# EternalEvan/InstaRevive

Measured on AMD Instinct MI355X. Metric: 512->2048 one-step SR images/sec, higher is better.
Workload: dtype bf16

## Files before the change

### instarevive_amd/csrc/conv_s1.hip

```cpp
#include <stdlib.h>
#include <type_traits>
#include <utility>
#include "agpr256.h"
#include "common.h"
#include "kernels.h"
#include "conv_s1_epi.h"

namespace cs1 {
constexpr int TH = 16, TW = 32, HWD = TW + 2, HP = (TH + 2) * HWD;
constexpr int BK = 32, ROWB = 64;
constexpr int H_Q = (HP + 15) / 16;
constexpr int HALO_BYTES = H_Q * 1024;
constexpr int H_I = 10;
constexpr int BN = 128, WT_BYTES = BN * ROWB;
constexpr int NSB = 4;
constexpr int NHB = 3;
constexpr int W_OFF = NHB * HALO_BYTES;
constexpr int LDS_MAIN = W_OFF + NSB * WT_BYTES;
static_assert(cs1e::BYTES <= HALO_BYTES, "epilogue slabs + reduction area must fit one halo buffer");
constexpr int LDS_BYTES = LDS_MAIN;
template <int NTAP>
struct Geo {
    static constexpr int K = NTAP == 9 ? 3 : 2, HWD = TW + K - 1, HP = (TH + K - 1) * HWD, H_Q = (HP + 15) / 16, H_I = (H_Q + 3) / 4;
};
static_assert(Geo<9>::H_Q == H_Q && Geo<9>::H_I == H_I && Geo<4>::H_Q == 36 && Geo<4>::H_I == 9, "halo piece counts");
constexpr int nh(int ntap, int t) { return ntap == 9 ? (t < 4 ? 2 : (t < 6 ? 1 : 0)) : (t == 0 ? 3 : 2); }
constexpr int nh_first(int ntap, int t) { return ntap == 9 ? (t < 4 ? 2 * t : (t < 6 ? 4 + t : 0)) : (t == 0 ? 0 : 1 + 2 * t); }
constexpr int hkey(int hx) { return ((hx >> 2) & 1) << 1; }
}

#ifdef IR_S1_STAMPS
__device__ unsigned long long g_s1_stamps[1024 * 8];
#define IR_S1_T(v) const unsigned long long v = __builtin_amdgcn_s_memrealtime()
#define IR_S1_ACC(k, a, b) do { if (tid == 0) g_s1_stamps[blockIdx.x * 8 + (k)] += (b) - (a); } while (0)
#else
#define IR_S1_T(v) do { } while (0)
#define IR_S1_ACC(k, a, b) do { } while (0)
#endif

typedef __attribute__((address_space(3))) void* cs1_lds_t;
template <int LO>
IR_DEVINL void cs1_mfma(bf16x8 w, bf16x8 px) {
    asm volatile("v_mfma_f32_16x16x32_bf16 a[%c2:%c3], %0, %1, a[%c2:%c3]" ::"v"(w), "v"(px), "n"(LO), "n"(LO + 3));
}

template <int UP, int NTAP, bool NORM = false, int EFULL = 0>
__global__ __launch_bounds__(256, 1) void conv_halo_s1_kernel(IGemmParams p, int tiles_y, int tiles_x, int total_vb) {
    static_assert(!NORM || (UP == 0 && NTAP == 9), "the in-kernel GroupNorm form exists for the plain 9-tap conv");
#if defined(__HIP_DEVICE_COMPILE__)
    using namespace cs1;
    using G = Geo<NTAP>;
    constexpr int K = G::K, HWD = G::HWD, HP = G::HP, H_Q = G::H_Q, H_I = G::H_I;
    constexpr bool PH = NTAP == 4;
    constexpr int NP_OFF = LDS_MAIN, NP_SLOT = 2 * 512 * 4;
    __shared__ __attribute__((aligned(1024))) unsigned char smem[NORM ? LDS_MAIN + 2 * NP_SLOT : LDS_BYTES];
    const int tid = threadIdx.x, lane = tid & 63, wid = tid >> 6;
    const int wu = __builtin_amdgcn_readfirstlane(wid);
    const int c16 = lane & 15, kq = lane >> 4;
    const int NT = p.Cout_pad / BN;
    const int MT = p.NB * tiles_y * tiles_x * (PH ? 4 : 1);
    const int Hc = UP ? 2 * p.H : p.H, Wc = UP ? 2 * p.W : p.W;
    const int chunks = p.Cin / BK;

    struct Tile { int img, trem, oy0, ox0, n0, dy, dx; };
    auto decode = [&](int bid, Tile& t) -> bool {
        const int xcd = bid & 7, jb = bid >> 3;
        const int mt = (jb / NT) * 8 + xcd, nt = jb % NT;
        if (bid >= total_vb || mt >= MT) return false;
        t.n0 = nt * BN;
        const int per_img = tiles_y * tiles_x * (PH ? 4 : 1);
        t.img = mt / per_img;
        t.trem = mt - t.img * per_img;
        const int ph = PH ? (t.trem & 3) : 0, tile = PH ? (t.trem >> 2) : t.trem;
        t.dy = ph >> 1; t.dx = ph & 1;
        const int ty = tile / tiles_x, tx = tile - ty * tiles_x;
        t.oy0 = ty * TH; t.ox0 = tx * TW;
        return true;
    };
    constexpr uint32_t OOB = 0xfffffff0u;
    auto tile_base = [&](const Tile& t) -> const bf16_t* {
        const int by = max(t.oy0 - 1 + t.dy, 0) >> UP;
        return p.in + ((long)t.img * p.H + by) * p.W * p.in_cs;
    };
    auto describe = [&](const Tile& t, uint32_t (&hp)[H_I], uint32_t (&wp)[2]) {
        const int by = max(t.oy0 - 1 + t.dy, 0) >> UP;
#pragma unroll
        for (int i = 0; i < H_I; ++i) {
            const int q = min(wu + 4 * i, H_Q - 1);
            const int hpix = q * 16 + (lane >> 2);
            const int hy = hpix / HWD, hx = hpix - hy * HWD;
            const int cy = t.oy0 + hy - 1 + t.dy, cx = t.ox0 + hx - 1 + t.dx;
            const bool ok = hpix < HP && cy >= 0 && cy < Hc && cx >= 0 && cx < Wc;
            const int iy = min(max(cy, 0), Hc - 1) >> UP, ix = min(max(cx, 0), Wc - 1) >> UP;
            const uint32_t sw = (uint32_t)((lane & 3) ^ hkey(hx));
            hp[i] = ok ? (uint32_t)(((iy - by) * p.W + ix) * p.in_cs) * 2u + sw * 16u : OOB;
        }
#pragma unroll
        for (int i = 0; i < 2; ++i) {
            const int row = (wu + 4 * i) * 16 + (lane >> 2);
            wp[i] = (uint32_t)(((PH ? (2 * t.dy + t.dx) * p.Cout_pad : 0) + t.n0 + row) * (int)p.wgt_rs) * 2u + (uint32_t)((lane & 3) ^ hkey(row)) * 16u;
        }
    };
    auto rsrc_of = [&](const void* base) { return __builtin_amdgcn_make_buffer_rsrc(const_cast<void*>(base), 0, 0x7fffffff, 0x00020000); };
    const __amdgpu_buffer_rsrc_t w_rsrc = rsrc_of(p.wgt);
    const uint32_t lds0 = lds_addr(smem);
    uint32_t hrd[K];
#pragma unroll
    for (int kx = 0; kx < K; ++kx) {
        const int hx = kx + c16;
        hrd[kx] = lds0 + ((4 * wid) * HWD + hx) * ROWB + ((kq ^ hkey(hx)) << 4);
    }
    const uint32_t wrd = lds0 + W_OFF + c16 * ROWB + ((kq ^ hkey(c16)) << 4);
    bf16x8 fw[2][8], fp[NORM ? 1 : 2][NORM ? 1 : 8];
    bf16x8 fq[3];

    Tile cur, nxt;
    int bid = blockIdx.x;
    while (bid < total_vb && !decode(bid, cur)) bid += gridDim.x;
    if (bid >= total_vb) return;
    uint32_t h_ptr[H_I], h_nxt[H_I], w_ptr[2], w_nxt[2];
    describe(cur, h_ptr, w_ptr);
    const bf16_t* base_cur = tile_base(cur);
    const bf16_t* base_nxt = base_cur;

    auto halo_issue = [&](auto ic, int ci, int buf) {
        constexpr int i = decltype(ic)::value;
        const int q = min(wu + 4 * i, H_Q - 1);
        const bool mine = ci < chunks;
        __builtin_amdgcn_raw_ptr_buffer_load_lds(rsrc_of(mine ? base_cur : base_nxt), (cs1_lds_t)(smem + buf * HALO_BYTES + q * 1024), 16,
                                                 (int)(mine ? h_ptr[i] : h_nxt[i]), (mine ? ci : ci - chunks) * (BK * 2), 0, 0);
    };
    auto w_issue = [&](int chunk, int tap, bool mine, int slot) {
        const int koff = tap * p.Cin + chunk * BK;
#pragma unroll
        for (int i = 0; i < 2; ++i)
            __builtin_amdgcn_raw_ptr_buffer_load_lds(w_rsrc, (cs1_lds_t)(smem + W_OFF + slot * WT_BYTES + (wu + 4 * i) * 1024), 16,
                                                     (int)(mine ? w_ptr[i] : w_nxt[i]), koff * 2, 0, 0);
    };

    int hb3 = 0;
    [&]<int... I>(std::integer_sequence<int, I...>) { (halo_issue(std::integral_constant<int, I>{}, 0, 0), ...); }(std::make_integer_sequence<int, H_I>{});
#pragma unroll
    for (int t = 0; t < NSB; ++t) w_issue(0, t, true, t);
    [&]<int... I>(std::integer_sequence<int, I...>) { (halo_issue(std::integral_constant<int, I>{}, 1, 1), ...); }(std::make_integer_sequence<int, H_I>{});

    auto step = [&](auto tc, auto setc, int c, int hbuf) {
        constexpr int T = decltype(tc)::value, SET = decltype(setc)::value;
        constexpr int TNX = (T + 1) % NTAP, KXN = TNX % K, KYN = TNX / K;
        const int s = c * NTAP + T;
        const uint32_t hb = (uint32_t)(T == NTAP - 1 ? (hbuf == 2 ? 0 : hbuf + 1) : hbuf) * HALO_BYTES;
        const int hfill = hbuf == 0 ? 2 : hbuf - 1;
        const uint32_t ha = hrd[KXN] + hb;
        const uint32_t wa = wrd + (uint32_t)((s + 1) & 3) * WT_BYTES;
        constexpr int TW4 = (T + 4) % NTAP;
        int cw = c + (T + 4) / NTAP, tw = TW4;
        const bool wmine = cw < chunks;
        if (!wmine) cw = 0;
        const bool hmine = c + 2 < chunks;
        const int hoff = (hmine ? c + 2 : c + 2 - chunks) * (BK * 2);
        const int wkoff = (tw * p.Cin + cw * BK) * 2;
        auto halo_piece = [&](auto kc) {
            constexpr int KP = decltype(kc)::value;
            constexpr int PI = nh(NTAP, T) > KP ? nh_first(NTAP, T) + KP : 0;
            const int q = min(wu + 4 * PI, H_Q - 1);
            __builtin_amdgcn_raw_ptr_buffer_load_lds(rsrc_of(hmine ? base_cur : base_nxt), (cs1_lds_t)(smem + hfill * HALO_BYTES + q * 1024), 16,
                                                     (int)(hmine ? h_ptr[PI] : h_nxt[PI]), hoff, 0, 0);
        };
        [&]<int... I>(std::integer_sequence<int, I...>) {
            ([&] {
                constexpr int PT = I >> 3, CT = I & 7;
                if constexpr ((I & 3) == 0) {
                    constexpr int R = I >> 2;
                    if constexpr (R < 8) fw[SET ^ 1][R] = lds_read16<R * 1024>(wa);
                    else fp[SET ^ 1][R - 8] = lds_read16<(((R - 8) >> 1) + KYN) * HWD * ROWB + ((R - 8) & 1) * 1024>(ha);
                }
                __builtin_amdgcn_sched_barrier(0);
                cs1_mfma<4 * I>(fw[SET][CT], fp[SET][PT]);
                __builtin_amdgcn_sched_barrier(0);
                if constexpr (I == 1 && nh(NTAP, T) > 0) {
                    halo_piece(std::integral_constant<int, 0>{});
                    __builtin_amdgcn_sched_barrier(0);
                }
                if constexpr (I == 5 && nh(NTAP, T) > 1) {
                    halo_piece(std::integral_constant<int, 1>{});
                    __builtin_amdgcn_sched_barrier(0);
                }
                if constexpr (I == 17 && nh(NTAP, T) > 2) {
                    halo_piece(std::integral_constant<int, 2>{});
                    __builtin_amdgcn_sched_barrier(0);
                }
                if constexpr (I == 10 || I == 13) {
                    constexpr int K = I == 10 ? 0 : 1;
                    __builtin_amdgcn_raw_ptr_buffer_load_lds(w_rsrc, (cs1_lds_t)(smem + W_OFF + (s & 3) * WT_BYTES + (wu + 4 * K) * 1024), 16,
                                                             (int)(wmine ? w_ptr[K] : w_nxt[K]), wkoff, 0, 0);
                    __builtin_amdgcn_sched_barrier(0);
                }
            }(), ...);
        }(std::make_integer_sequence<int, 64>{});
        wait_lds<0>();
        wait_vm<4 + nh(NTAP, (T + NTAP - 1) % NTAP) + nh(NTAP, T)>();
        __builtin_amdgcn_sched_barrier(0);
        __builtin_amdgcn_s_barrier();
        __builtin_amdgcn_sched_barrier(0);
    };

    int tpar = 0;
    bool first_tile = true;
    uint32_t nkm = 0;
    if constexpr (NORM) {
#pragma unroll
        for (int i = 0; i < H_I; ++i) {
            const int hpix = min(wu + 4 * i, H_Q - 1) * 16 + (lane >> 2);
            nkm |= (uint32_t)(hkey(hpix % HWD) >> 1) << i;
        }
    }
    float nsc[NORM ? 8 : 1], nsh[NORM ? 8 : 1];
    auto load_tab = [&](int slot, int img) {
        float* tab = reinterpret_cast<float*>(smem + NP_OFF + slot * NP_SLOT);
        for (int i = tid; i < p.Cin; i += 256) {
            tab[i] = p.nrm_scale[(long)img * p.Cin + i];
            tab[512 + i] = p.nrm_shift[(long)img * p.Cin + i];
        }
    };
    typedef float nf32x2 __attribute__((ext_vector_type(2)));
    nf32x2 nfa[NORM ? 4 : 1], nfe[NORM ? 4 : 1];
    auto sfma = [](float a, float b, float c) { float r; asm("v_fma_f32 %0, %1, %2, %3" : "=v"(r) : "v"(a), "v"(b), "v"(c)); return r; };
    auto smul = [](float a, float b) { float r; asm("v_mul_f32 %0, %1, %2" : "=v"(r) : "v"(a), "v"(b)); return r; };
    auto sadd1 = [](float a) { float r; asm("v_add_f32 %0, 1.0, %1" : "=v"(r) : "v"(a)); return r; };
    auto norm_stage = [&](auto stc, const bf16x8& raw, uint4& out) {
        constexpr int ST = decltype(stc)::value;
        if constexpr (ST == 0) {
            bf16x8 rw = raw;
            asm volatile("s_waitcnt lgkmcnt(2)" : "+v"(rw));
            const uint4 u = __builtin_bit_cast(uint4, rw);
            const uint32_t w[4] = {u.x, u.y, u.z, u.w};
#pragma unroll
            for (int e = 0; e < 4; ++e) {
                nfa[e] = nf32x2{sfma(bflo(w[e]), nsc[2 * e], nsh[2 * e]), sfma(bfhi(w[e]), nsc[2 * e + 1], nsh[2 * e + 1])};
            }
        } else if constexpr (ST == 1 || ST == 2) {
#pragma unroll
            for (int e = 2 * (ST - 1); e < 2 * ST; ++e) {
                const nf32x2 t = nf32x2{smul(nfa[e][0], -1.44269504088896340736f), smul(nfa[e][1], -1.44269504088896340736f)};
                nfe[e] = nf32x2{__builtin_amdgcn_exp2f(t[0]), __builtin_amdgcn_exp2f(t[1])};
            }
        } else if constexpr (ST == 3 || ST == 4) {
#pragma unroll
            for (int e = 2 * (ST - 3); e < 2 * (ST - 2); ++e) {
                const nf32x2 d = nf32x2{sadd1(nfe[e][0]), sadd1(nfe[e][1])};
                nfe[e] = nf32x2{fast_rcp(d[0]), fast_rcp(d[1])};
            }
        } else {
            nf32x2 y[4];
#pragma unroll
            for (int e = 0; e < 4; ++e) y[e] = nf32x2{smul(nfa[e][0], nfe[e][0]), smul(nfa[e][1], nfe[e][1])};
            out = make_uint4(pack2bf_valu(y[0][0], y[0][1]), pack2bf_valu(y[1][0], y[1][1]), pack2bf_valu(y[2][0], y[2][1]), pack2bf_valu(y[3][0], y[3][1]));
        }
    };
    auto step_n = [&](auto tc, auto setc, int c, int hbuf) {
        constexpr int T = decltype(tc)::value, SET = decltype(setc)::value;
        constexpr int KX = T % K, KY = T / K;
        constexpr int TNX = (T + 1) % NTAP, KXN = TNX % K, KYN = TNX / K;
        const int s = c * NTAP + T;
        const uint32_t hbc = (uint32_t)hbuf * HALO_BYTES;
        const uint32_t hbn = (uint32_t)(T == NTAP - 1 ? (hbuf == 2 ? 0 : hbuf + 1) : hbuf) * HALO_BYTES;
        const int hfill = hbuf == 0 ? 2 : hbuf - 1;
        const uint32_t ha_c = hrd[KX] + hbc, ha_n = hrd[KXN] + hbn;
        const uint32_t wa = wrd + (uint32_t)((s + 1) & 3) * WT_BYTES;
        constexpr int TW4 = (T + 4) % NTAP;
        int cw = c + (T + 4) / NTAP, tw = TW4;
        const bool wmine = cw < chunks;
        if (!wmine) cw = 0;
        const bool hmine = c + 2 < chunks;
        const int hoff = (hmine ? c + 2 : c + 2 - chunks) * (BK * 2);
        const int wkoff = (tw * p.Cin + cw * BK) * 2;
        auto halo_piece = [&](auto kc) {
            constexpr int KP = decltype(kc)::value;
            constexpr int PI = nh(NTAP, T) > KP ? nh_first(NTAP, T) + KP : 0;
            const int q = min(wu + 4 * PI, H_Q - 1);
            __builtin_amdgcn_raw_ptr_buffer_load_lds(rsrc_of(hmine ? base_cur : base_nxt), (cs1_lds_t)(smem + hfill * HALO_BYTES + q * 1024), 16,
                                                     (int)(hmine ? h_ptr[PI] : h_nxt[PI]), hoff, 0, 0);
        };
        const bool nx = c + 1 >= chunks;
        const uint32_t nbuf = lds0 + (uint32_t)(hbuf == 2 ? 0 : hbuf + 1) * HALO_BYTES;
        constexpr int NU = T < 6 ? 1 : (T < 8 ? 2 : 0);
        constexpr int UI[2] = {T < 8 ? T : 0, T == 6 ? 8 : 9};
        constexpr int RD[2] = {NU == 2 ? 6 : 22, 30}, WR[2] = {NU == 2 ? 31 : 48, 56};
        bf16x8 nraw;
        uint4 nout;
        auto unit_addr = [&](int i) { return nbuf + (uint32_t)(wu + 4 * i) * 1024u + (uint32_t)((lane ^ (((nkm >> i) & 1u) << 1)) * 16); };
        auto unit_ok = [&](int i) { return wu + 4 * i < H_Q && (nx ? h_nxt[i] : h_ptr[i]) != OOB; };
        [&]<int... I>(std::integer_sequence<int, I...>) {
            ([&] {
                constexpr int PT = I >> 3, CT = I & 7, G8 = I >> 3;
                if constexpr ((I & 7) == 0) {
                    if constexpr (I > 0) wait_lds<3>();
                    constexpr int P2 = G8 + 2;
                    if constexpr (P2 < 8) fq[(P2 + 2 * T) % 3] = lds_read16<((P2 >> 1) + KY) * HWD * ROWB + (P2 & 1) * 1024>(ha_c);
                    else fq[((P2 - 8) + 2 * TNX) % 3] = lds_read16<(((P2 - 8) >> 1) + KYN) * HWD * ROWB + ((P2 - 8) & 1) * 1024>(ha_n);
                }
                if constexpr ((I & 7) == 2) fw[SET ^ 1][G8] = lds_read16<G8 * 1024>(wa);
                __builtin_amdgcn_sched_barrier(0);
                cs1_mfma<4 * I>(fw[SET][CT], fq[(PT + 2 * T) % 3]);
                __builtin_amdgcn_sched_barrier(0);
                if constexpr (I == 1 && nh(NTAP, T) > 0) { halo_piece(std::integral_constant<int, 0>{}); __builtin_amdgcn_sched_barrier(0); }
                if constexpr (I == 5 && nh(NTAP, T) > 1) { halo_piece(std::integral_constant<int, 1>{}); __builtin_amdgcn_sched_barrier(0); }
                if constexpr (I == 17 && nh(NTAP, T) > 2) { halo_piece(std::integral_constant<int, 2>{}); __builtin_amdgcn_sched_barrier(0); }
                if constexpr (I == 10 || I == 13) {
                    constexpr int KW = I == 10 ? 0 : 1;
                    __builtin_amdgcn_raw_ptr_buffer_load_lds(w_rsrc, (cs1_lds_t)(smem + W_OFF + (s & 3) * WT_BYTES + (wu + 4 * KW) * 1024), 16,
                                                             (int)(wmine ? w_ptr[KW] : w_nxt[KW]), wkoff, 0, 0);
                    __builtin_amdgcn_sched_barrier(0);
                }
                constexpr int II = I;
                [&]<int... UU>(std::integer_sequence<int, UU...>) {
                    ([&] {
                        constexpr int U = UU;
                        if constexpr (U < NU) {
                            if constexpr (II == RD[U]) {
                                nraw = lds_read16<0>(unit_addr(UI[U])); __builtin_amdgcn_sched_barrier(0); }
                            if constexpr (II >= RD[U] + 8 && II <= RD[U] + 23 && (II - RD[U] - 8) % 3 == 0) {
                                norm_stage(std::integral_constant<int, (II - RD[U] - 8) / 3>{}, nraw, nout);
                                __builtin_amdgcn_sched_barrier(0);
                            }
                            if constexpr (II == WR[U]) {
                                typedef unsigned int nu32x4 __attribute__((ext_vector_type(4)));
                                const nu32x4 o = {nout.x, nout.y, nout.z, nout.w};
                                if (unit_ok(UI[U])) asm volatile("ds_write_b128 %0, %1" ::"v"(unit_addr(UI[U])), "v"(o) : "memory");
                                __builtin_amdgcn_sched_barrier(0);
                            }
                        }
                    }(), ...);
                }(std::integer_sequence<int, 0, 1>{});
            }(), ...);
        }(std::make_integer_sequence<int, 64>{});
        wait_lds<0>();
        wait_vm<4 + nh(NTAP, (T + NTAP - 1) % NTAP) + nh(NTAP, T)>();
        __builtin_amdgcn_sched_barrier(0);
        if constexpr (T == NTAP - 1) if (c + 1 < chunks) {
            const int c2 = c + 2;
            const float* tab = reinterpret_cast<const float*>(smem + NP_OFF + ((c2 < chunks ? tpar : tpar ^ 1) * NP_SLOT)) + (c2 < chunks ? c2 : c2 - chunks) * BK + (lane & 3) * 8;
#pragma unroll
            for (int e = 0; e < 8; ++e) { nsc[e] = tab[e]; nsh[e] = tab[512 + e]; }
        }
        __builtin_amdgcn_s_barrier();
        __builtin_amdgcn_sched_barrier(0);
    };

    for (;;) {
        IR_S1_T(st0);
        int nbid = bid + gridDim.x;
        while (nbid < total_vb && !decode(nbid, nxt)) nbid += gridDim.x;
        const bool more = nbid < total_vb;
        if (!more) nxt = cur;
        describe(nxt, h_nxt, w_nxt);
        base_nxt = tile_base(nxt);
        if constexpr (NORM) {
            if (first_tile) load_tab(tpar, cur.img);
            load_tab(tpar ^ 1, nxt.img);
        }
        if constexpr (EFULL != 0) {
            [&]<int... CT>(std::integer_sequence<int, CT...>) {
                ([&] {
                    const f32x4 b4 = p.bias ? *reinterpret_cast<const f32x4*>(p.bias + cur.n0 + 16 * CT + 4 * kq) : f32x4{0.f, 0.f, 0.f, 0.f};
                    if constexpr (CT == 0)
                        asm volatile(".set ir_cs1_i, 0\n\t.rept 8\n\tv_accvgpr_write_b32 a[ir_cs1_i], %0\n\tv_accvgpr_write_b32 a[ir_cs1_i + 1], %1\n\t"
                                     "v_accvgpr_write_b32 a[ir_cs1_i + 2], %2\n\tv_accvgpr_write_b32 a[ir_cs1_i + 3], %3\n\t.set ir_cs1_i, ir_cs1_i + 32\n\t.endr"
                                     ::"v"(b4[0]), "v"(b4[1]), "v"(b4[2]), "v"(b4[3]) : IR_AGPR256_CLOBBERS);
                    else
                        asm volatile(".set ir_cs1_i, %c4\n\t.rept 8\n\tv_accvgpr_write_b32 a[ir_cs1_i], %0\n\tv_accvgpr_write_b32 a[ir_cs1_i + 1], %1\n\t"
                                     "v_accvgpr_write_b32 a[ir_cs1_i + 2], %2\n\tv_accvgpr_write_b32 a[ir_cs1_i + 3], %3\n\t.set ir_cs1_i, ir_cs1_i + 32\n\t.endr"
                                     ::"v"(b4[0]), "v"(b4[1]), "v"(b4[2]), "v"(b4[3]), "n"(4 * CT));
                }(), ...);
            }(std::make_integer_sequence<int, 8>{});
        } else {
            asm volatile(".set ir_cs1_i, 0\n\t.rept 256\n\tv_accvgpr_write_b32 a[ir_cs1_i], 0\n\t.set ir_cs1_i, ir_cs1_i + 1\n\t.endr" ::: IR_AGPR256_CLOBBERS);
        }
        wait_dma();
        __syncthreads();
        if constexpr (NORM) {
            if (first_tile) {
                const float* tab = reinterpret_cast<const float*>(smem + NP_OFF + tpar * NP_SLOT) + (lane & 3) * 8;
#pragma unroll
                for (int e = 0; e < 8; ++e) { nsc[e] = tab[e]; nsh[e] = tab[512 + e]; }
                for (int i = 0; i < H_I; ++i) {
                    if (wu + 4 * i >= H_Q || h_ptr[i] == OOB) continue;
                    uint4* v = reinterpret_cast<uint4*>(smem + hb3 * HALO_BYTES + (wu + 4 * i) * 1024 + ((lane ^ (((nkm >> i) & 1u) << 1)) * 16));
                    const uint4 u = *v;
                    const uint32_t w[4] = {u.x, u.y, u.z, u.w};
                    uint32_t o[4];
#pragma unroll
                    for (int e = 0; e < 4; ++e) o[e] = pack2bf_valu(silu(bflo(w[e]) * nsc[2 * e] + nsh[2 * e]), silu(bfhi(w[e]) * nsc[2 * e + 1] + nsh[2 * e + 1]));
                    *v = make_uint4(o[0], o[1], o[2], o[3]);
                }
                __syncthreads();
                first_tile = false;
            }
            const float* tab1 = reinterpret_cast<const float*>(smem + NP_OFF + tpar * NP_SLOT) + BK + (lane & 3) * 8;
#pragma unroll
            for (int e = 0; e < 8; ++e) { nsc[e] = tab1[e]; nsh[e] = tab1[512 + e]; }
        }
        if constexpr (NORM) {
            [&]<int... R>(std::integer_sequence<int, R...>) { ((fw[0][R] = lds_read16<R * 1024>(wrd)), ...); }(std::make_integer_sequence<int, 8>{});
            fq[0] = lds_read16<0>(hrd[0] + (uint32_t)hb3 * HALO_BYTES);
            fq[1] = lds_read16<1024>(hrd[0] + (uint32_t)hb3 * HALO_BYTES);
        } else {
        [&]<int... R>(std::integer_sequence<int, R...>) {
            ([&] {
                if constexpr (R < 8) fw[0][R] = lds_read16<R * 1024>(wrd);
                else fp[0][R - 8] = lds_read16<((R - 8) >> 1) * HWD * ROWB + ((R - 8) & 1) * 1024>(hrd[0] + (uint32_t)hb3 * HALO_BYTES);
            }(), ...);
        }(std::make_integer_sequence<int, 16>{});
        }
        wait_lds<0>();
        IR_S1_T(st1);
#ifdef IR_S1_STAMPS
        const unsigned long long sc0 = __builtin_amdgcn_s_memtime();
#endif
        for (int c = 0; c < chunks; c += 2) {
            const int hb3b = hb3 == 2 ? 0 : hb3 + 1;
            if constexpr (NORM) {
                [&]<int... U>(std::integer_sequence<int, U...>) { (step_n(std::integral_constant<int, U>{}, std::integral_constant<int, (U & 1)>{}, c, hb3), ...); }(std::make_integer_sequence<int, NTAP>{});
                [&]<int... U>(std::integer_sequence<int, U...>) { (step_n(std::integral_constant<int, U>{}, std::integral_constant<int, ((U + NTAP) & 1)>{}, c + 1, hb3b), ...); }(std::make_integer_sequence<int, NTAP>{});
            } else {
            [&]<int... U>(std::integer_sequence<int, U...>) { (step(std::integral_constant<int, U>{}, std::integral_constant<int, (U & 1)>{}, c, hb3), ...); }(std::make_integer_sequence<int, NTAP>{});
            [&]<int... U>(std::integer_sequence<int, U...>) { (step(std::integral_constant<int, U>{}, std::integral_constant<int, ((U + NTAP) & 1)>{}, c + 1, hb3b), ...); }(std::make_integer_sequence<int, NTAP>{});
            }
            hb3 = hb3b == 2 ? 0 : hb3b + 1;
        }

        IR_S1_T(st2);
#ifdef IR_S1_STAMPS
        if (tid == 0) g_s1_stamps[blockIdx.x * 8 + 5] += __builtin_amdgcn_s_memtime() - sc0;
#endif
        asm volatile("s_nop 15\n\ts_nop 7" ::: "memory");
        IR_S1_T(st3);
        unsigned char* ebuf = smem + (hb3 == 0 ? 2 : hb3 - 1) * HALO_BYTES;
#ifdef IR_S1_STAMPS
        unsigned long long st4v = 0;
        cs1_epilogue<false, EFULL>(p, ebuf, tid, lane, wid, c16, kq, cur.n0, cur.img, cur.oy0, cur.ox0, cur.trem, &st4v,
                            PH ? 2 : 1, cur.dy, cur.dx, PH ? p.H : p.Ho, PH ? p.W : p.Wo);
        const unsigned long long st4 = st4v;
#else
        cs1_epilogue<false, EFULL>(p, ebuf, tid, lane, wid, c16, kq, cur.n0, cur.img, cur.oy0, cur.ox0, cur.trem, nullptr,
                            PH ? 2 : 1, cur.dy, cur.dx, PH ? p.H : p.Ho, PH ? p.W : p.Wo);
#endif
        IR_S1_T(st5);
        IR_S1_ACC(0, st0, st1); IR_S1_ACC(1, st1, st2); IR_S1_ACC(2, st2, st3); IR_S1_ACC(3, st3, st4); IR_S1_ACC(4, st4, st5);
#ifdef IR_S1_STAMPS
        if (tid == 0) g_s1_stamps[blockIdx.x * 8 + 6] += 1;
#endif
        if (!more) break;
        tpar ^= 1;
        bid = nbid;
        cur = nxt;
        base_cur = base_nxt;
#pragma unroll
        for (int i = 0; i < H_I; ++i) h_ptr[i] = h_nxt[i];
        w_ptr[0] = w_nxt[0]; w_ptr[1] = w_nxt[1];
    }
    wait_dma();
#endif
}

bool ir_conv_s1_takes(const IGemmParams& p) {
    if (g_ir_plain_kernels || p.fp8 || p.force_generic) return false;
    if (p.taps != 9 || p.stride != 1 || p.pad != 1 || (p.Cin & 127)) return false;
    if (p.Cout != p.Cout_pad || p.Cout_pad % 128) return false;
    if (p.act != IR_ACT_NONE || p.gate || p.out2 || p.out_f32) return false;
    if (p.res && (p.res_f32 || p.res_mod > 0 || (p.res_cs & 7) || (reinterpret_cast<uintptr_t>(p.res) & 15))) return false;
    if ((p.out_cs & 7) || (reinterpret_cast<uintptr_t>(p.out) & 15)) return false;
    if (p.bias && (reinterpret_cast<uintptr_t>(p.bias) & 15)) return false;
    const long tiles = (long)((p.Ho + 15) / 16) * ((p.Wo + 31) / 32) * (p.Cout_pad / 128);
    return tiles >= (p.s1_min_tiles > 32 ? p.s1_min_tiles : 32);
}
int ir_conv_s1_tiles(const IGemmParams& p) { return ((p.Ho + 15) / 16) * ((p.Wo + 31) / 32); }

static int cs1_cus() {
    static const int cus = [] {
        int dev = 0, n = 0;
        if (hipGetDevice(&dev) != hipSuccess || hipDeviceGetAttribute(&n, hipDeviceAttributeMultiprocessorCount, dev) != hipSuccess || n < 8) n = 256;
        return n & ~7;
    }();
    return cus;
}

bool ir_conv_s1_norm_takes(const IGemmParams& p) {
    static const bool off = getenv("IR_NO_S1_NORM") != nullptr;
    return !off && p.nrm_scale && p.nrm_shift && !p.up && !p.up2x2 && p.Cin <= 512 && ir_conv_s1_takes(p);
}

int ir_launch_conv_s1(const IGemmParams& p, hipStream_t s) {
    if (!ir_conv_s1_takes(p)) return -2;
    if ((p.nrm_scale || p.nrm_shift) && !ir_conv_s1_norm_takes(p)) return -16;
    if (p.gn_part && (p.gn_cpg < 4 || p.gn_cpg > 32 || (p.gn_cpg & (p.gn_cpg - 1)) || p.gn_chunks != ir_conv_s1_tiles(p))) return -13;
    const int tiles_y = (p.Ho + 15) / 16, tiles_x = (p.Wo + 31) / 32;
    const long MT = (long)p.NB * tiles_y * tiles_x, NT = p.Cout_pad / 128;
    const long total = ((MT + 7) / 8) * 8 * NT;
    if (total > 0x7fffffffL) return -12;
    const long grid = total < cs1_cus() ? total : cs1_cus();
    const int full = (p.Ho % 16 == 0 && p.Wo % 32 == 0 && p.out_scale == 1.f) ? (p.gn_part ? 1 : 2) : 0;
    const dim3 g((unsigned)grid), b(256);
    if (p.nrm_scale) {
        if (full == 1) hipLaunchKernelGGL((conv_halo_s1_kernel<0, 9, true, 1>), g, b, 0, s, p, tiles_y, tiles_x, (int)total);
        else if (full == 2) hipLaunchKernelGGL((conv_halo_s1_kernel<0, 9, true, 2>), g, b, 0, s, p, tiles_y, tiles_x, (int)total);
        else hipLaunchKernelGGL((conv_halo_s1_kernel<0, 9, true>), g, b, 0, s, p, tiles_y, tiles_x, (int)total);
    } else if (p.up) hipLaunchKernelGGL((conv_halo_s1_kernel<1, 9>), g, b, 0, s, p, tiles_y, tiles_x, (int)total);
    else if (full == 1) hipLaunchKernelGGL((conv_halo_s1_kernel<0, 9, false, 1>), g, b, 0, s, p, tiles_y, tiles_x, (int)total);
    else if (full == 2) hipLaunchKernelGGL((conv_halo_s1_kernel<0, 9, false, 2>), g, b, 0, s, p, tiles_y, tiles_x, (int)total);
    else hipLaunchKernelGGL((conv_halo_s1_kernel<0, 9>), g, b, 0, s, p, tiles_y, tiles_x, (int)total);
    return hipGetLastError() == hipSuccess ? 0 : -1;
}

bool ir_conv_s1_up2x2_takes(const IGemmParams& pin) {
    static const bool off = getenv("IR_NO_UP2X2") != nullptr;
    if (off || !pin.up || pin.res) return false;
    IGemmParams p = pin;
    p.up = 0; p.Ho = pin.H; p.Wo = pin.W;
    if (!ir_conv_s1_takes(p)) return false;
    return 4L * ((pin.H + 15) / 16) * ((pin.W + 31) / 32) * (pin.Cout_pad / 128) >= 32;
}
int ir_conv_s1_up2x2_tiles(const IGemmParams& p) { return 4 * ((p.H + 15) / 16) * ((p.W + 31) / 32); }

int ir_launch_conv_s1_up2x2(const IGemmParams& p, hipStream_t s) {
    if (!ir_conv_s1_up2x2_takes(p)) return -2;
    if (p.wgt_rs != 4L * p.Cin || p.Ho != 2 * p.H || p.Wo != 2 * p.W) return -3;
    if (p.gn_part && (p.gn_cpg < 4 || p.gn_cpg > 32 || (p.gn_cpg & (p.gn_cpg - 1)) || p.gn_chunks != ir_conv_s1_up2x2_tiles(p))) return -13;
    const int tiles_y = (p.H + 15) / 16, tiles_x = (p.W + 31) / 32;
    const long MT = (long)p.NB * 4 * tiles_y * tiles_x, NT = p.Cout_pad / 128;
    const long total = ((MT + 7) / 8) * 8 * NT;
    if (total > 0x7fffffffL) return -12;
    const long grid = total < cs1_cus() ? total : cs1_cus();
    if (p.gn_part && p.H % 16 == 0 && p.W % 32 == 0 && p.out_scale == 1.f) hipLaunchKernelGGL((conv_halo_s1_kernel<0, 4, false, 1>), dim3((unsigned)grid), dim3(256), 0, s, p, tiles_y, tiles_x, (int)total);
    else hipLaunchKernelGGL((conv_halo_s1_kernel<0, 4>), dim3((unsigned)grid), dim3(256), 0, s, p, tiles_y, tiles_x, (int)total);
    return hipGetLastError() == hipSuccess ? 0 : -1;
}
```

### instarevive_amd/csrc/conv_s1_epi.h

```cpp
#pragma once
#include "common.h"
#include "kernels.h"

namespace cs1e {
constexpr int SROW = 132;
constexpr int SLAB = 16 * SROW * 4;
constexpr int RED_OFF = 4 * SLAB;
constexpr int BYTES = RED_OFF + 4 * 16 * 16;
}

template <int I>
IR_DEVINL float cs1_acc_read() {
    float x;
    asm volatile("v_accvgpr_read_b32 %0, a[%c1]" : "=v"(x) : "n"(I));
    return x;
}

template <bool GATE, bool FULL, bool FGN>
IR_DEVINL void cs1_epilogue_impl(const IGemmParams& p, unsigned char* ebuf, int tid, int lane, int wid, int c16, int kq, int t_n0, int t_img, int t_oy0,
                                 int t_ox0, int t_trem, unsigned long long* mid_stamp, int omul, int oyoff, int oxoff, int hlim,
                                 int wlim) {
    using namespace cs1e;
    float* slab = reinterpret_cast<float*>(ebuf + wid * SLAB);
    const int co8 = (lane & 15) * 8, xq = lane >> 4;
    const int n0 = t_n0, img = t_img, oy0 = t_oy0, ox0 = t_ox0;
    const float osc = p.out_scale;
    constexpr bool BIAS_IN_ACC = FULL && !GATE;
    f32x4 bias4[(GATE || BIAS_IN_ACC) ? 1 : 8], g_lo, g_hi, b_lo, b_hi;
    if constexpr (BIAS_IN_ACC) {
    } else if constexpr (GATE) {
        g_lo = *reinterpret_cast<const f32x4*>(p.gate + n0 + co8);
        g_hi = *reinterpret_cast<const f32x4*>(p.gate + n0 + co8 + 4);
        b_lo = (p.bias ? *reinterpret_cast<const f32x4*>(p.bias + n0 + co8) : f32x4{0.f, 0.f, 0.f, 0.f}) * g_lo;
        b_hi = (p.bias ? *reinterpret_cast<const f32x4*>(p.bias + n0 + co8 + 4) : f32x4{0.f, 0.f, 0.f, 0.f}) * g_hi;
    } else {
#pragma unroll
        for (int ct = 0; ct < 8; ++ct)
            bias4[ct] = (p.bias ? *reinterpret_cast<const f32x4*>(p.bias + n0 + 16 * ct + 4 * kq) : f32x4{0.f, 0.f, 0.f, 0.f}) * osc;
    }
    f32x4 sA4 = {0.f, 0.f, 0.f, 0.f}, qA4 = sA4, sB4 = sA4, qB4 = sA4;
    const int oyw = oy0 + 4 * wid, oxl = ox0 + xq;
    unsigned xm = 0;
    if constexpr (!FULL) {
#pragma unroll
        for (int it = 0; it < 8; ++it) xm |= (oxl + 4 * it < wlim ? 1u : 0u) << it;
    }
    const long pix0 = ((long)img * p.Ho + (long)omul * oyw + oyoff) * p.Wo + (long)omul * oxl + oxoff;
    bf16_t* obase = reinterpret_cast<bf16_t*>(p.out) + pix0 * p.out_cs + n0 + co8;
    const bf16_t* rbase = reinterpret_cast<const bf16_t*>(p.res) + pix0 * p.res_cs + n0 + co8;
    const bf16_t* rsafe = reinterpret_cast<const bf16_t*>(p.res) + (((long)img * p.Ho + (long)omul * oy0 + oyoff) * p.Wo + (long)omul * ox0 + oxoff) * p.res_cs + n0 + co8;
    const long o_row = (long)omul * p.Wo * p.out_cs, r_row = (long)omul * p.Wo * p.res_cs;
    const long o_col = (long)omul * p.out_cs, r_col = (long)omul * p.res_cs;
    const long upix = ((long)img * p.Ho + (long)omul * oyw + oyoff) * p.Wo + (long)omul * ox0 + oxoff;
    bf16_t* const uo = reinterpret_cast<bf16_t*>(p.out) + upix * p.out_cs + n0;
    const bf16_t* const ur = reinterpret_cast<const bf16_t*>(p.res) + upix * p.res_cs + n0;
    unsigned lo_o = (unsigned)(xq * (int)o_col + co8) * 2u, lo_r = (unsigned)(xq * (int)r_col + co8) * 2u;
    if constexpr (FULL) asm volatile("" : "+v"(lo_o), "+v"(lo_r));
    const unsigned uo_row = (unsigned)o_row * 2u, ur_row = (unsigned)r_row * 2u, uo_c4 = 8u * (unsigned)o_col, ur_c4 = 8u * (unsigned)r_col;
    unsigned char* const uob = reinterpret_cast<unsigned char*>(uo);
    const unsigned char* const urb = reinterpret_cast<const unsigned char*>(ur);
    constexpr bool GN = FULL && FGN;
    const bool do_gn = FULL ? FGN : p.gn_part != nullptr;
    uint4 rrb[2][8];
    auto res_fetch = [&](int a) {
        if constexpr (FULL) {
#pragma unroll
            for (int it = 0; it < 8; ++it) rrb[a & 1][it] = *reinterpret_cast<const uint4*>(urb + (lo_r + (unsigned)a * ur_row + (unsigned)it * ur_c4));
        } else {
            const bool yok = oyw + a < hlim;
#pragma unroll
            for (int it = 0; it < 8; ++it) {
                const bool v = yok && ((xm >> it) & 1);
                rrb[a & 1][it] = *reinterpret_cast<const uint4*>(v ? rbase + a * r_row + (long)(4 * it) * r_col : rsafe);
            }
        }
    };
    auto pass = [&](auto ac, auto resc) {
        constexpr int A = decltype(ac)::value;
        constexpr bool RES = decltype(resc)::value;
        const bool yok = FULL || oyw + A < hlim;
        uint4 (&rr)[8] = rrb[A & 1];
        if constexpr (RES && A < 3) res_fetch(A + 1);
        [&]<int... MXS>(std::integer_sequence<int, MXS...>) {
            ([&] {
                constexpr int MX = MXS;
                [&]<int... CTS>(std::integer_sequence<int, CTS...>) {
                    ([&] {
                        constexpr int CT = CTS, LO = 4 * ((A * 2 + MX) * 8 + CT);
                        f32x4 v = f32x4{cs1_acc_read<LO>(), cs1_acc_read<LO + 1>(), cs1_acc_read<LO + 2>(), cs1_acc_read<LO + 3>()};
                        if constexpr (!GATE && !BIAS_IN_ACC) v = v * osc + bias4[CT];
                        *reinterpret_cast<f32x4*>(&slab[c16 * SROW + 16 * CT + 4 * kq]) = v;
                    }(), ...);
                }(std::make_integer_sequence<int, 8>{});
                if constexpr (FULL) __builtin_amdgcn_sched_barrier(0);
                __builtin_amdgcn_fence(__ATOMIC_RELEASE, "wavefront");
                __builtin_amdgcn_wave_barrier();
                __builtin_amdgcn_fence(__ATOMIC_ACQUIRE, "wavefront");
                f32x4 lo[4], hi[4];
#pragma unroll
                for (int j = 0; j < 4; ++j) {
                    lo[j] = *reinterpret_cast<const f32x4*>(&slab[(4 * j + xq) * SROW + co8]);
                    hi[j] = *reinterpret_cast<const f32x4*>(&slab[(4 * j + xq) * SROW + co8 + 4]);
                }
#pragma unroll
                for (int j = 0; j < 4; ++j) {
                    const int it = 4 * MX + j;
                    f32x4 a = lo[j], b = hi[j];
                    if constexpr (GATE) { a = a * g_lo + b_lo; b = b * g_hi + b_hi; }
                    if constexpr (RES) {
                        a += f32x4{bflo(rr[it].x), bfhi(rr[it].x), bflo(rr[it].y), bfhi(rr[it].y)};
                        b += f32x4{bflo(rr[it].z), bfhi(rr[it].z), bflo(rr[it].w), bfhi(rr[it].w)};
                    }
                    const uint4 pk = make_uint4(pack2bf_valu(a[0], a[1]), pack2bf_valu(a[2], a[3]), pack2bf_valu(b[0], b[1]), pack2bf_valu(b[2], b[3]));
                    if constexpr (FULL) {
                        *reinterpret_cast<uint4*>(uob + (lo_o + (unsigned)A * uo_row + (unsigned)it * uo_c4)) = pk;
                        if constexpr (GN) {
                            const f32x4 ar = {bflo(pk.x), bfhi(pk.x), bflo(pk.y), bfhi(pk.y)}, br = {bflo(pk.z), bfhi(pk.z), bflo(pk.w), bfhi(pk.w)};
                            sA4 += ar; qA4 += ar * ar;
                            sB4 += br; qB4 += br * br;
                        }
                        __builtin_amdgcn_sched_barrier(0);
                    } else if (yok && ((xm >> it) & 1)) {
                        *reinterpret_cast<uint4*>(obase + A * o_row + (long)(4 * it) * o_col) = pk;
                        if (do_gn) {
                            const f32x4 ar = {bflo(pk.x), bfhi(pk.x), bflo(pk.y), bfhi(pk.y)}, br = {bflo(pk.z), bfhi(pk.z), bflo(pk.w), bfhi(pk.w)};
                            sA4 += ar; qA4 += ar * ar;
                            sB4 += br; qB4 += br * br;
                        }
                    }
                }
                __builtin_amdgcn_fence(__ATOMIC_RELEASE, "wavefront");
                __builtin_amdgcn_wave_barrier();
                __builtin_amdgcn_fence(__ATOMIC_ACQUIRE, "wavefront");
                if constexpr (FULL) __builtin_amdgcn_sched_barrier(0);
            }(), ...);
        }(std::make_integer_sequence<int, 2>{});
    };
    if (p.res) {
        res_fetch(0);
        pass(std::integral_constant<int, 0>{}, std::true_type{});
        pass(std::integral_constant<int, 1>{}, std::true_type{});
        pass(std::integral_constant<int, 2>{}, std::true_type{});
        pass(std::integral_constant<int, 3>{}, std::true_type{});
    } else {
        pass(std::integral_constant<int, 0>{}, std::false_type{});
        pass(std::integral_constant<int, 1>{}, std::false_type{});
        pass(std::integral_constant<int, 2>{}, std::false_type{});
        pass(std::integral_constant<int, 3>{}, std::false_type{});
    }
    if (mid_stamp) *mid_stamp = __builtin_amdgcn_s_memrealtime();
    if (do_gn) {
        const float sA = (sA4[0] + sA4[1]) + (sA4[2] + sA4[3]), qA = (qA4[0] + qA4[1]) + (qA4[2] + qA4[3]);
        const float sB = (sB4[0] + sB4[1]) + (sB4[2] + sB4[3]), qB = (qB4[0] + qB4[1]) + (qB4[2] + qB4[3]);
        f32x4 v = {sA, qA, sB, qB};
#pragma unroll
        for (int e = 0; e < 4; ++e) {
            v[e] += __shfl_xor(v[e], 16);
            v[e] += __shfl_xor(v[e], 32);
        }
        float* red = reinterpret_cast<float*>(ebuf + RED_OFF);
        if (lane < 16) *reinterpret_cast<f32x4*>(&red[(wid * 16 + lane) * 4]) = v;
        __syncthreads();
        if (tid < 32) {
            const int L = tid >> 1, hf = (tid & 1) * 2;
            float a = (red[(0 * 16 + L) * 4 + hf] + red[(1 * 16 + L) * 4 + hf]) + (red[(2 * 16 + L) * 4 + hf] + red[(3 * 16 + L) * 4 + hf]);
            float b = (red[(0 * 16 + L) * 4 + hf + 1] + red[(1 * 16 + L) * 4 + hf + 1]) + (red[(2 * 16 + L) * 4 + hf + 1] + red[(3 * 16 + L) * 4 + hf + 1]);
            const int upg = p.gn_cpg >> 2;
            for (int m = 1; m < upg; m <<= 1) {
                a += __shfl_xor(a, m);
                b += __shfl_xor(b, m);
            }
            if ((tid & (upg - 1)) == 0) {
                const int G = p.Cout / p.gn_cpg, g = n0 / p.gn_cpg + tid / upg;
                float* dst = p.gn_part + ((long)img * p.gn_chunks + t_trem) * 2 * G;
                dst[g] = a;
                dst[G + g] = b;
            }
        }
    }
}

template <bool GATE, int EMODE = 0>
IR_DEVINL void cs1_epilogue(const IGemmParams& p, unsigned char* ebuf, int tid, int lane, int wid, int c16, int kq, int t_n0, int t_img, int t_oy0,
                            int t_ox0, int t_trem, unsigned long long* mid_stamp, int omul, int oyoff, int oxoff, int hlim,
                            int wlim) {
    cs1_epilogue_impl<GATE, EMODE != 0, EMODE == 1>(p, ebuf, tid, lane, wid, c16, kq, t_n0, t_img, t_oy0, t_ox0, t_trem, mid_stamp, omul, oyoff, oxoff, hlim, wlim);
}
```

Baseline: 8.713.

## Prefetch bias and norm tables into LDS via async DMA to avoid full drain

```diff
diff --git a/instarevive_amd/csrc/conv_s1.hip b/instarevive_amd/csrc/conv_s1.hip
--- a/instarevive_amd/csrc/conv_s1.hip
+++ b/instarevive_amd/csrc/conv_s1.hip
@@ -53,7 +53,8 @@
     constexpr int K = G::K, HWD = G::HWD, HP = G::HP, H_Q = G::H_Q, H_I = G::H_I;
     constexpr bool PH = NTAP == 4;
     constexpr int NP_OFF = LDS_MAIN, NP_SLOT = 2 * 512 * 4;
-    __shared__ __attribute__((aligned(1024))) unsigned char smem[NORM ? LDS_MAIN + 2 * NP_SLOT : LDS_BYTES];
+    constexpr int BT_OFF = NORM ? LDS_MAIN + 2 * NP_SLOT : LDS_BYTES;
+    __shared__ __attribute__((aligned(1024))) unsigned char smem[BT_OFF + (EFULL != 0 ? 2 * BN * 4 : 0)];
     const int tid = threadIdx.x, lane = tid & 63, wid = tid >> 6;
     const int wu = __builtin_amdgcn_readfirstlane(wid);
     const int c16 = lane & 15, kq = lane >> 4;
@@ -118,6 +119,17 @@
     int bid = blockIdx.x;
     while (bid < total_vb && !decode(bid, cur)) bid += gridDim.x;
     if (bid >= total_vb) return;
+    float* const btab = reinterpret_cast<float*>(smem + BT_OFF);
+    int bpar = 0;
+    if constexpr (EFULL != 0) {
+        if (tid < BN) btab[tid] = p.bias ? p.bias[cur.n0 + tid] : 0.f;
+        __syncthreads();
+    }
+    auto load_bias = [&](int slot, int n0) {
+        if (wu >= 2)
+            __builtin_amdgcn_raw_ptr_buffer_load_lds(__builtin_amdgcn_make_buffer_rsrc(const_cast<float*>(p.bias), 0, p.bias ? 0x7fffffff : 0, 0x00020000),
+                                                     (cs1_lds_t)(smem + BT_OFF + slot * BN * 4 + (wu - 2) * 256), 4, (n0 + (wu - 2) * 64 + lane) * 4, 0, 0, 0);
+    };
     uint32_t h_ptr[H_I], h_nxt[H_I], w_ptr[2], w_nxt[2];
     describe(cur, h_ptr, w_ptr);
     const bf16_t* base_cur = tile_base(cur);
@@ -144,6 +156,14 @@
     for (int t = 0; t < NSB; ++t) w_issue(0, t, true, t);
     [&]<int... I>(std::integer_sequence<int, I...>) { (halo_issue(std::integral_constant<int, I>{}, 1, 1), ...); }(std::make_integer_sequence<int, H_I>{});
 
+    bool first_tile = true;
+    auto step_wait = [&](auto tc, int c) {
+        constexpr int T = decltype(tc)::value, N = 4 + nh(NTAP, (T + NTAP - 1) % NTAP) + nh(NTAP, T);
+        if constexpr (EFULL != 0 && T == 0) {
+            if (c == 0 && !first_tile) { wait_vm<2 + nh(NTAP, 0) + 32>(); return; }
+        }
+        wait_vm<N>();
+    };
     auto step = [&](auto tc, auto setc, int c, int hbuf) {
         constexpr int T = decltype(tc)::value, SET = decltype(setc)::value;
         constexpr int TNX = (T + 1) % NTAP, KXN = TNX % K, KYN = TNX / K;
@@ -198,14 +218,13 @@
             }(), ...);
         }(std::make_integer_sequence<int, 64>{});
         wait_lds<0>();
-        wait_vm<4 + nh(NTAP, (T + NTAP - 1) % NTAP) + nh(NTAP, T)>();
+        step_wait(tc, c);
         __builtin_amdgcn_sched_barrier(0);
         __builtin_amdgcn_s_barrier();
         __builtin_amdgcn_sched_barrier(0);
     };
 
     int tpar = 0;
-    bool first_tile = true;
     uint32_t nkm = 0;
     if constexpr (NORM) {
 #pragma unroll
@@ -216,10 +235,12 @@
     }
     float nsc[NORM ? 8 : 1], nsh[NORM ? 8 : 1];
     auto load_tab = [&](int slot, int img) {
-        float* tab = reinterpret_cast<float*>(smem + NP_OFF + slot * NP_SLOT);
-        for (int i = tid; i < p.Cin; i += 256) {
-            tab[i] = p.nrm_scale[(long)img * p.Cin + i];
-            tab[512 + i] = p.nrm_shift[(long)img * p.Cin + i];
+        const int np = p.Cin >> 6;
+        for (int j = wu; j < 2 * np; j += 4) {
+            const bool sh = j >= np;
+            const int jj = sh ? j - np : j;
+            __builtin_amdgcn_raw_ptr_buffer_load_lds(rsrc_of(sh ? p.nrm_shift : p.nrm_scale), (cs1_lds_t)(smem + NP_OFF + slot * NP_SLOT + (sh ? 2048 : 0) + jj * 256), 4,
+                                                     (int)((img * p.Cin + jj * 64 + lane) * 4), 0, 0, 0);
         }
     };
     typedef float nf32x2 __attribute__((ext_vector_type(2)));
@@ -335,7 +356,7 @@
             }(), ...);
         }(std::make_integer_sequence<int, 64>{});
         wait_lds<0>();
-        wait_vm<4 + nh(NTAP, (T + NTAP - 1) % NTAP) + nh(NTAP, T)>();
+        step_wait(tc, c);
         __builtin_amdgcn_sched_barrier(0);
         if constexpr (T == NTAP - 1) if (c + 1 < chunks) {
             const int c2 = c + 2;
@@ -356,13 +377,15 @@
         describe(nxt, h_nxt, w_nxt);
         base_nxt = tile_base(nxt);
         if constexpr (NORM) {
-            if (first_tile) load_tab(tpar, cur.img);
-            load_tab(tpar ^ 1, nxt.img);
+            if (first_tile) {
+                load_tab(tpar, cur.img);
+                load_tab(tpar ^ 1, nxt.img);
+            }
         }
         if constexpr (EFULL != 0) {
             [&]<int... CT>(std::integer_sequence<int, CT...>) {
                 ([&] {
-                    const f32x4 b4 = p.bias ? *reinterpret_cast<const f32x4*>(p.bias + cur.n0 + 16 * CT + 4 * kq) : f32x4{0.f, 0.f, 0.f, 0.f};
+                    const f32x4 b4 = *reinterpret_cast<const f32x4*>(btab + bpar * BN + 16 * CT + 4 * kq);
                     if constexpr (CT == 0)
                         asm volatile(".set ir_cs1_i, 0\n\t.rept 8\n\tv_accvgpr_write_b32 a[ir_cs1_i], %0\n\tv_accvgpr_write_b32 a[ir_cs1_i + 1], %1\n\t"
                                      "v_accvgpr_write_b32 a[ir_cs1_i + 2], %2\n\tv_accvgpr_write_b32 a[ir_cs1_i + 3], %3\n\t.set ir_cs1_i, ir_cs1_i + 32\n\t.endr"
@@ -376,8 +399,17 @@
         } else {
             asm volatile(".set ir_cs1_i, 0\n\t.rept 256\n\tv_accvgpr_write_b32 a[ir_cs1_i], 0\n\t.set ir_cs1_i, ir_cs1_i + 1\n\t.endr" ::: IR_AGPR256_CLOBBERS);
         }
-        wait_dma();
-        __syncthreads();
+        if (EFULL != 0 && !first_tile) {
+            wait_vm<32>();
+            if constexpr (NORM) load_tab(tpar ^ 1, nxt.img);
+            load_bias(bpar ^ 1, nxt.n0);
+            asm volatile("s_waitcnt lgkmcnt(0)\n\ts_barrier" ::: "memory");
+        } else {
+            if constexpr (EFULL != 0) load_bias(bpar ^ 1, nxt.n0);
+            if constexpr (NORM) if (!first_tile) load_tab(tpar ^ 1, nxt.img);
+            wait_dma();
+            __syncthreads();
+        }
         if constexpr (NORM) {
             if (first_tile) {
                 const float* tab = reinterpret_cast<const float*>(smem + NP_OFF + tpar * NP_SLOT) + (lane & 3) * 8;
@@ -394,7 +426,6 @@
                     *v = make_uint4(o[0], o[1], o[2], o[3]);
                 }
                 __syncthreads();
-                first_tile = false;
             }
             const float* tab1 = reinterpret_cast<const float*>(smem + NP_OFF + tpar * NP_SLOT) + BK + (lane & 3) * 8;
 #pragma unroll
@@ -451,7 +482,9 @@
         if (tid == 0) g_s1_stamps[blockIdx.x * 8 + 6] += 1;
 #endif
         if (!more) break;
+        first_tile = false;
         tpar ^= 1;
+        bpar ^= 1;
         bid = nbid;
         cur = nxt;
         base_cur = base_nxt;
diff --git a/instarevive_amd/csrc/conv_s1_epi.h b/instarevive_amd/csrc/conv_s1_epi.h
--- a/instarevive_amd/csrc/conv_s1_epi.h
+++ b/instarevive_amd/csrc/conv_s1_epi.h
@@ -160,7 +160,7 @@
         }
         float* red = reinterpret_cast<float*>(ebuf + RED_OFF);
         if (lane < 16) *reinterpret_cast<f32x4*>(&red[(wid * 16 + lane) * 4]) = v;
-        __syncthreads();
+        asm volatile("s_waitcnt lgkmcnt(0)\n\ts_barrier" ::: "memory");
         if (tid < 32) {
             const int L = tid >> 1, hf = (tid & 1) * 2;
             float a = (red[(0 * 16 + L) * 4 + hf] + red[(1 * 16 + L) * 4 + hf]) + (red[(2 * 16 + L) * 4 + hf] + red[(3 * 16 + L) * 4 + hf]);
```

After: 8.756 (median of 6 runs). About the same (+0.5%).
